# kwohlfahrt/collision

Measured on AMD Instinct MI355X. Metric: M spheres/sec end-to-end (bounds->Morton->radix sort->LBVH->refit->traversal), higher is better.
Workload: dtype f32 coords / u32 keys+ids; 1 GPU; BASELINE config 2: 1000000 uniform-random spheres, r=0.001, f32, RandomState(4), pair capacity 131072; spheres_total=1000000, group_size=256, parallelism=single

## Files before the change

### collision_amd/csrc/bvh.hip

```cpp
#include "col_common.h"
#include <math.h>

namespace {

constexpr u32 END = 0xFFFFFFFFu;

template <typename T> struct BTypes;
template <> struct BTypes<float> {
    typedef float4 V4;
    typedef uint32_t Bits;
    struct alignas(4) V3 { float x, y, z; };
};
template <> struct BTypes<double> {
    typedef double4 V4;
    typedef uint64_t Bits;
    struct alignas(8) V3 { double x, y, z; };
};

template <typename T> __device__ __forceinline__ u32 link_load(const T *bounds, uint64_t row) {
    typedef typename BTypes<T>::Bits Bits;
    return (u32) reinterpret_cast<const Bits *>(bounds)[row * 4 + 3];
}
template <typename T> __device__ __forceinline__ void link_store(T *bounds, uint64_t row, u32 v) {
    typedef typename BTypes<T>::Bits Bits;
// ... 1076 lines not shown
    if (coord_bytes != 4 && coord_bytes != 8) return COL_EINVAL;
    if (n_dev && !partials) return COL_EINVAL;
    if (partials && (parts == 0 || parts > COL_MINMAX_PARTS)) return COL_EINVAL;
    if (padded < n || (capacity > 0 && !pairs)) return COL_EINVAL;
    if (!scratch) return COL_ENOSCRATCH;
    if (col_radix_tile_override_active()) return COL_EINVAL;
    hipStream_t s = col_stream(stream);
    if (n == 0) {
        COL_HIP(hipMemsetAsync(counter, 0, sizeof(uint32_t), s));
        return COL_OK;
    }
    (void)flags;
    char *p = (char *)scratch;
    void *range = p;           p += 256;
    void *red_scratch = p;     p += col_reduce_scratch_bytes(coord_bytes == 8 ? COL_F64 : COL_F32, 4);
    p = (char *)(((uintptr_t)p + 255) & ~(uintptr_t)255);
    void *sort_scratch = p;    p += col_radix_scratch_bytes(padded, 4, 4);
    p = (char *)(((uintptr_t)p + 255) & ~(uintptr_t)255);
    void *lbvh_scratch = p;    p += col_lbvh_scratch_bytes(n, coord_bytes);
    p = (char *)(((uintptr_t)p + 255) & ~(uintptr_t)255);
    void *packed = p;          p += (size_t)n * 4 * coord_bytes;
    p = (char *)(((uintptr_t)p + 255) & ~(uintptr_t)255);
    void *chunk_hdr = p;       p += sizeof(ChunkHdr) + 256 + 8 * ((size_t)n / 64 + 1) + 256;
    p = (char *)(((uintptr_t)p + 255) & ~(uintptr_t)255);
    uint32_t *msd_fused = (uint32_t *)p;
    const bool chunked = (sort_plan & COL_TRAVERSE_CHUNKED) != 0;
    sort_plan &= 1;
    uint32_t *publish = oversize ? oversize + 2 : nullptr;
    int rc;
    uint32_t *report_word = nullptr;
    const uint32_t tile = col_radix_tile(padded, 4, 4);
    if (tile == 1024 || tile == 4096 || tile == 8192) {
        const bool msd = sort_plan == COL_SORT_MSD && padded <= COL_MSD_MAX_N;
        const uint32_t nsums = msd ? (uint32_t)(col_radix_msd_fused_bytes() / sizeof(uint32_t)) : 0u;
        if (msd && col_ceil_div(padded, tile) > (uint64_t)COL_MSD_GROUP * COL_MSD_GROUPS) return COL_EINVAL;
        if (!partials) {
            if ((rc = col_minmax4_stage1_zero(stream, coords, n, coord_bytes, red_scratch, &parts, msd_fused, nsums))) return rc;
            partials = red_scratch;
        } else if (msd)
            COL_HIP(hipMemsetAsync(msd_fused, 0, nsums * sizeof(uint32_t), s));
        if ((rc = col_morton_tile(stream, coords, radii, partials, parts, n, padded, coord_bytes, codes0, ids0, packed,
                                  counter, (uint32_t *)sort_scratch, tile, (uint32_t)col_ceil_div(padded, tile), msd ? 22 : 0,
                                  publish, n_dev, msd ? msd_fused : nullptr))) return rc;
        if (msd) rc = col_radix_sort_msd_fused(stream, codes0, codes1, ids0, ids1, padded, sort_scratch, oversize, n_dev, msd_fused);
        else rc = col_radix_sort_ex(stream, codes0, codes1, ids0, ids1, padded, 4, 4, sort_scratch, 0, 1);
        if (rc) return rc;
        if (!msd && oversize && padded <= COL_MSD_MAX_N) report_word = oversize + 1;
    } else {
        if (n_dev) return COL_EINVAL;
        if ((rc = col_reduce(stream, coords, n, coord_bytes == 8 ? COL_F64 : COL_F32, 4, COL_OP_MINMAX, red_scratch, range))) return rc;
        if ((rc = col_morton_ex(stream, coords, radii, range, n, padded, coord_bytes, codes0, ids0, packed, counter, publish))) return rc;
        if ((rc = col_radix_sort(stream, codes0, codes1, ids0, ids1, padded, 4, 4, sort_scratch, 0))) return rc;
    }
    uint32_t *sched = (!chunked && (n >= COL_DYNAMIC_PACKETS_FROM || (g_traverse_variant & 32768))) ? (uint32_t *)((char *)chunk_hdr + sizeof(ChunkHdr)) : nullptr;
    const int order_mode = chunked || col_lbvh_order_forced() ? 1 : 0;
    uint32_t *walk_order = n > 256 && (chunked || (sched && (n <= COL_DEAL_MAX_N || order_mode))) ? (uint32_t *)((char *)chunk_hdr + sizeof(ChunkHdr) + 256) : nullptr;
    if ((rc = col_lbvh_ex(stream, codes1, ids1, coords, radii, packed, nodes, bounds, lbvh_scratch, n, coord_bytes,
                          chunked ? (uint32_t *)chunk_hdr : sched, n_dev, walk_order, order_mode, chunked ? 16u : 8u, report_word, padded))) return rc;
    if (chunked) return traverse_chunked_dev(stream, pairs, counter, capacity, nodes, bounds, n, coord_bytes, chunk_hdr, n_dev, walk_order, true);
    if (n < 2) return COL_OK;
    if (coord_bytes == 4) return launch_traverse<float>(stream, pairs, counter, capacity, bounds, n, nullptr, 0, sched, n_dev, walk_order);
    return launch_traverse<double>(stream, pairs, counter, capacity, bounds, n, nullptr, 0, sched, n_dev, walk_order);
}

}
```

### collision_amd/csrc/col_common.h

```cpp
#pragma once
#include <hip/hip_runtime.h>
#include <stdint.h>
#include "../../include/collision_hip.h"
#include "../../include/collision_hip_debug.h"

#define COL_WAVE 64

#define COL_HIP(expr)                                  \
    do {                                               \
        hipError_t e_ = (expr);                        \
        if (e_ != hipSuccess) return (int)e_;          \
    } while (0)

#define COL_LAUNCH_OK()                                \
    do {                                               \
        hipError_t e_ = hipGetLastError();             \
        if (e_ != hipSuccess) return (int)e_;          \
    } while (0)

extern "C" int col_morton_ex(void *stream, const void *coords, const void *radii, const void *range, uint32_t n,
                             uint32_t padded, int coord_bytes, uint32_t *codes, uint32_t *ids, void *packed,
                             uint32_t *zero_word, uint32_t *publish);
extern "C" int col_lbvh_ex(void *stream, const uint32_t *codes, const uint32_t *ids, const void *coords, const void *radii,
                           const void *packed, col_node *nodes, void *bounds, void *scratch, uint32_t n, int coord_bytes,
                           uint32_t *zero8,
                           const uint32_t *n_dev,
                           uint32_t *walk_order,
                           int order_mode,
                           uint32_t nzero = 8,
                           uint32_t *report_word = nullptr,
                           uint32_t report_n = 0);
extern "C" int col_radix_sort_msd_dev(void *stream, const uint32_t *keys, uint32_t *keys_out, const uint32_t *vals, uint32_t *vals_out,
                                      uint64_t n, void *scratch, uint32_t *oversize, const uint32_t *n_real_dev);

#define COL_MINMAX_PARTS 256
#define COL_REGION_BOXES 8
#define COL_MSD_SMALL_N 1900000u
#define COL_MSD_MAX_N 4050000u
extern "C" int col_minmax4_stage1(void *stream, const void *rows, uint64_t n, int coord_bytes, void *partials, uint32_t *parts);
extern "C" int col_minmax4_stage1_dev(void *stream, const void *rows, const uint32_t *n_dev, uint32_t n_max, int coord_bytes,
                                      void *partials, uint32_t *parts);
extern "C" int col_morton_tile(void *stream, const void *coords, const void *radii, const void *partials, uint32_t parts,
                               uint32_t n, uint32_t padded, int coord_bytes, uint32_t *codes, uint32_t *ids, void *packed,
                               uint32_t *zero_word, uint32_t *hist0, uint32_t tile, uint32_t nblocks, int hist_shift,
                               uint32_t *publish, const uint32_t *n_dev, uint32_t *gsum);
#define COL_MSD_GROUP 32u
#define COL_MSD_GROUPS 32u
extern "C" int col_minmax4_stage1_zero(void *stream, const void *rows, uint64_t n, int coord_bytes, void *partials, uint32_t *parts,
                                       uint32_t *zero, uint32_t nzero);
extern "C" size_t col_radix_msd_fused_bytes(void);
extern "C" int col_radix_sort_msd_fused(void *stream, const uint32_t *keys, uint32_t *keys_out, const uint32_t *vals, uint32_t *vals_out,
                                        uint64_t n, void *scratch, uint32_t *oversize, const uint32_t *n_real_dev, uint32_t *fused);
extern "C" int col_radix_sort_ex(void *stream, const void *keys, void *keys_out, const void *vals, void *vals_out,
                                 uint64_t n, int key_bytes, int val_bytes, void *scratch, int copy_back, int have_hist0);

extern "C" int col_traverse_ghost_packets(void *stream, uint32_t *pairs, uint32_t *counter, uint32_t capacity, const void *bounds,
                                          uint32_t n, int coord_bytes, const uint32_t *rec, const uint32_t *order,
                                          const uint32_t *count, uint32_t max_ghosts, const uint32_t *local_gids,
                                          const uint32_t *n_dev);
extern "C" int col_radix_sort_low_passes(void *stream, const uint32_t *keys, uint32_t *keys_out, const uint32_t *vals,
                                         uint32_t *vals_out, uint64_t n, void *scratch, int passes);
extern "C" int col_radix_bucket_report(void *stream, const uint32_t *sorted_codes, uint64_t n, uint32_t *word);

static inline hipStream_t col_stream(void *s) { return (hipStream_t)s; }

static inline uint64_t col_ceil_div(uint64_t a, uint64_t b) { return (a + b - 1) / b; }

#ifdef __HIPCC__
typedef unsigned long long u64;
typedef unsigned int u32;
__device__ __forceinline__ void col_bucket_report_block(const u32 *__restrict__ sorted, u32 n, u32 *word, u32 *s_start) {
    const u32 d = threadIdx.x;
    const u32 want = d << 22;
    u32 lo = 0, hi = n;
    while (lo < hi) {
        const u32 mid = lo + ((hi - lo) >> 1);
        if (sorted[mid] < want) lo = mid + 1; else hi = mid;
    }
    s_start[d] = lo;
    if (d == 0) {
        u32 l2 = 0, h2 = n;
        while (l2 < h2) {
            const u32 mid = l2 + ((h2 - l2) >> 1);
            if (sorted[mid] < (1u << 30)) l2 = mid + 1; else h2 = mid;
        }
        s_start[256] = l2;
    }
    __syncthreads();
    u32 cnt = s_start[d + 1] - s_start[d];
#pragma unroll
    for (int o = COL_WAVE / 2; o > 0; o >>= 1) cnt = max(cnt, (u32)__shfl_xor((int)cnt, o, COL_WAVE));
    __syncthreads();
    if ((d & 63u) == 0) s_start[d >> 6] = cnt;
    __syncthreads();
    if (d == 0) {
        const u32 m = max(max(s_start[0], s_start[1]), max(s_start[2], s_start[3]));
        __hip_atomic_store(word, 0x80000000u | min(m, 0x7FFFFFFFu), __ATOMIC_RELAXED, __HIP_MEMORY_SCOPE_SYSTEM);
    }
}

__device__ __forceinline__ u32 lane_id() { return __lane_id(); }

__device__ __forceinline__ u32 count_of(u32 n, const u32 *__restrict__ n_dev) { return n_dev ? min(n, *n_dev) : n; }

__device__ __forceinline__ u32 mbcnt(u64 mask) {
    return __builtin_amdgcn_mbcnt_hi((u32)(mask >> 32), __builtin_amdgcn_mbcnt_lo((u32)mask, 0u));
}

__device__ __forceinline__ u32 wave_incl_scan(u32 v) {
    const u32 lane = lane_id();
#pragma unroll
    for (int o = 1; o < COL_WAVE; o <<= 1) {
        u32 t = __shfl_up(v, o, COL_WAVE);
        if (lane >= (u32)o) v += t;
    }
    return v;
}

__device__ __forceinline__ u32 wave_sum(u32 v) {
#pragma unroll
    for (int o = COL_WAVE / 2; o > 0; o >>= 1) v += __shfl_xor(v, o, COL_WAVE);
    return v;
}

template <int NT>
__device__ __forceinline__ u32 block_excl_scan(u32 v, u32 *warp_sums, u32 *total) {
    constexpr int NW = NT / COL_WAVE;
    const u32 lane = lane_id(), w = threadIdx.x / COL_WAVE;
    u32 incl = wave_incl_scan(v);
    if (lane == COL_WAVE - 1) warp_sums[w] = incl;
    __syncthreads();
    u32 base = 0, tot = 0;
#pragma unroll
    for (int i = 0; i < NW; i++) {
        u32 s = warp_sums[i];
        if ((u32)i < w) base += s;
        tot += s;
    }
    __syncthreads();
// ... 46 lines not shown
```

### collision_amd/csrc/morton.hip

```cpp
#include "col_common.h"

namespace {


template <typename T> struct alignas(4 * sizeof(T)) Vec4 { T x, y, z, w; };
template <> struct alignas(16) Vec4<double> { double x, y, z, w; };

__device__ __forceinline__ void publish_count(u32 *publish, u32 count) {
    if (publish) __hip_atomic_store(publish, 0x80000000u | (count < 0x7FFFFFFFu ? count : 0x7FFFFFFFu), __ATOMIC_RELAXED, __HIP_MEMORY_SCOPE_SYSTEM);
}

template <typename T>
__global__ __launch_bounds__(256) void k_morton(const Vec4<T> *__restrict__ coords,
                                                 const Vec4<T> *__restrict__ range, u32 n, u32 padded,
                                                 u32 *__restrict__ codes, u32 *__restrict__ ids,
                                                 const T *__restrict__ radii, Vec4<T> *__restrict__ packed,
                                                 u32 *__restrict__ zero_word, u32 *publish) {
    const u32 i = blockIdx.x * 256 + threadIdx.x;
    if (i == 0 && zero_word) {
        publish_count(publish, *zero_word);
        *zero_word = 0;
    }
    if (i >= padded) return;
    u32 code = 0xFFFFFFFFu;
    if (i < n) {
        const Vec4<T> mn = range[0], mx = range[1];
        const Vec4<T> c = coords[i];
        if (packed) {
            Vec4<T> pr = c;
            pr.w = radii[i];
            packed[i] = pr;
        }
        code = (expand_bits(quantize(c.x, mn.x, mx.x)) << 2) + (expand_bits(quantize(c.y, mn.y, mx.y)) << 1) +
               expand_bits(quantize(c.z, mn.z, mx.z));
    }
    codes[i] = code;
    if (ids) ids[i] = i;
}

constexpr int MT_ROWS = 4;
template <typename T, int NT, int HALVES>
__global__ __launch_bounds__(NT) void k_morton_tile(const Vec4<T> *__restrict__ coords, const T *__restrict__ partials,
                                                     u32 parts, u32 n_bound, u32 padded, u32 *__restrict__ codes,
                                                     u32 *__restrict__ ids, const T *__restrict__ radii,
                                                     Vec4<T> *__restrict__ packed, u32 *__restrict__ zero_word,
                                                     u32 *__restrict__ hist0, u32 nblocks, int hist_shift, u32 *publish,
                                                     const u32 *__restrict__ n_dev, u32 *__restrict__ gsum) {
    constexpr int TILE = NT * MT_ROWS * HALVES, NW = NT / 64;
    const u32 n = count_of(n_bound, n_dev);
    __shared__ T s_fold[NW][8];
    __shared__ u32 s_hist[256];
    const u32 tid = threadIdx.x, lane = tid & 63u, w = tid >> 6;
    if (blockIdx.x == 0 && tid == 0 && zero_word) {
        publish_count(publish, *zero_word);
        *zero_word = 0;
    }
    if (tid < 256) s_hist[tid] = 0;
    Vec4<T> c[MT_ROWS];
    T rad[MT_ROWS];
#pragma unroll
    for (int k = 0; k < MT_ROWS; k++) {
        const u32 i = blockIdx.x * TILE + k * NT + tid;
        if (i < n) {
            c[k] = coords[i];
            if (packed) rad[k] = radii[i];
        }
    }
    T acc[8];
#pragma unroll
    for (int k = 0; k < 4; k++) { acc[k] = (T)INFINITY; acc[4 + k] = -(T)INFINITY; }
    for (u32 i = tid; i < parts; i += NT) {
        const T *q = partials + (size_t)i * 8;
#pragma unroll
        for (int k = 0; k < 4; k++) {
            acc[k] = q[k] < acc[k] ? q[k] : acc[k];
            acc[4 + k] = q[4 + k] > acc[4 + k] ? q[4 + k] : acc[4 + k];
        }
    }
#pragma unroll
    for (int o = 32; o > 0; o >>= 1) {
#pragma unroll
        for (int k = 0; k < 4; k++) {
            const T lo = __shfl_xor(acc[k], o, 64), hi = __shfl_xor(acc[4 + k], o, 64);
            acc[k] = lo < acc[k] ? lo : acc[k];
            acc[4 + k] = hi > acc[4 + k] ? hi : acc[4 + k];
        }
    }
    if (lane == 0) {
#pragma unroll
        for (int k = 0; k < 8; k++) s_fold[w][k] = acc[k];
    }
    __syncthreads();
    Vec4<T> mn, mx;
    {
        T r[8];
#pragma unroll
        for (int k = 0; k < 8; k++) r[k] = s_fold[0][k];
        for (int ww = 1; ww < NW; ww++) {
#pragma unroll
            for (int k = 0; k < 4; k++) {
                r[k] = s_fold[ww][k] < r[k] ? s_fold[ww][k] : r[k];
                r[4 + k] = s_fold[ww][4 + k] > r[4 + k] ? s_fold[ww][4 + k] : r[4 + k];
            }
        }
        mn.x = r[0]; mn.y = r[1]; mn.z = r[2]; mn.w = r[3];
        mx.x = r[4]; mx.y = r[5]; mx.z = r[6]; mx.w = r[7];
    }
#pragma unroll
    for (int h = 0; h < HALVES; h++) {
        if (h > 0) {
#pragma unroll
            for (int k = 0; k < MT_ROWS; k++) {
                const u32 i = blockIdx.x * TILE + (h * MT_ROWS + k) * NT + tid;
                if (i < n) {
                    c[k] = coords[i];
                    if (packed) rad[k] = radii[i];
                }
            }
        }
#pragma unroll
        for (int k = 0; k < MT_ROWS; k++) {
            const u32 i = blockIdx.x * TILE + (h * MT_ROWS + k) * NT + tid;
            if (i >= padded) continue;
            u32 code = 0xFFFFFFFFu;
            if (i < n) {
                if (packed) {
                    Vec4<T> pr = c[k];
                    pr.w = rad[k];
                    packed[i] = pr;
                }
                code = (expand_bits(quantize(c[k].x, mn.x, mx.x)) << 2) + (expand_bits(quantize(c[k].y, mn.y, mx.y)) << 1) +
                       expand_bits(quantize(c[k].z, mn.z, mx.z));
            }
            codes[i] = code;
            if (ids) ids[i] = i;
            atomicAdd(&s_hist[(code >> hist_shift) & 255u], 1u);
        }
    }
    __syncthreads();
    if (gsum) {
        if (tid < 256) {
            const u32 c = s_hist[tid];
            hist0[(uint64_t)blockIdx.x * 256 + tid] = c;
            if (c) atomicAdd(&gsum[(blockIdx.x / COL_MSD_GROUP) * 256 + tid], c);
        }
        return;
    }
    if (tid < 256) hist0[(uint64_t)tid * nblocks + blockIdx.x] = s_hist[tid];
}

template <typename T>
int launch_morton_tile(hipStream_t s, u32 tile, const void *coords, const void *radii, const void *partials, uint32_t parts,
                       uint32_t n, uint32_t padded, uint32_t *codes, uint32_t *ids, void *packed, uint32_t *zero_word,
                       uint32_t *hist0, uint32_t nblocks, int hist_shift, uint32_t *publish, const uint32_t *n_dev, uint32_t *gsum) {
    dim3 grid(nblocks);
    if (tile == 1024)
        k_morton_tile<T, 256, 1><<<grid, dim3(256), 0, s>>>((const Vec4<T> *)coords, (const T *)partials, parts, n, padded, codes, ids,
                                                             (const T *)radii, (Vec4<T> *)packed, zero_word, hist0, nblocks, hist_shift, publish, n_dev, gsum);
    else if (tile == 4096)
        k_morton_tile<T, 1024, 1><<<grid, dim3(1024), 0, s>>>((const Vec4<T> *)coords, (const T *)partials, parts, n, padded, codes, ids,
                                                               (const T *)radii, (Vec4<T> *)packed, zero_word, hist0, nblocks, hist_shift, publish, n_dev, gsum);
    else
        k_morton_tile<T, 1024, 2><<<grid, dim3(1024), 0, s>>>((const Vec4<T> *)coords, (const T *)partials, parts, n, padded, codes, ids,
                                                               (const T *)radii, (Vec4<T> *)packed, zero_word, hist0, nblocks, hist_shift, publish, n_dev, gsum);
    COL_LAUNCH_OK();
    return COL_OK;
}

}

extern "C" {

int col_morton_tile(void *stream, const void *coords, const void *radii, const void *partials, uint32_t parts,
                    uint32_t n, uint32_t padded, int coord_bytes, uint32_t *codes, uint32_t *ids, void *packed,
                    uint32_t *zero_word, uint32_t *hist0, uint32_t tile, uint32_t nblocks, int hist_shift, uint32_t *publish,
                    const uint32_t *n_dev, uint32_t *gsum) {
    if (padded < n || parts == 0 || !hist0 || hist_shift < 0 || hist_shift > 24) return COL_EINVAL;
    if (tile != 1024 && tile != 4096 && tile != 8192) return COL_EINVAL;
    if (padded == 0) return COL_OK;
    if (packed && !radii) return COL_EINVAL;
    if (nblocks != (uint32_t)col_ceil_div(padded, tile)) return COL_EINVAL;
    if (coord_bytes == 4)
        return launch_morton_tile<float>(col_stream(stream), tile, coords, radii, partials, parts, n, padded, codes, ids, packed,
                                         zero_word, hist0, nblocks, hist_shift, publish, n_dev, gsum);
    if (coord_bytes == 8)
        return launch_morton_tile<double>(col_stream(stream), tile, coords, radii, partials, parts, n, padded, codes, ids, packed,
                                          zero_word, hist0, nblocks, hist_shift, publish, n_dev, gsum);
    return COL_EINVAL;
}

int col_morton_ex(void *stream, const void *coords, const void *radii, const void *range, uint32_t n, uint32_t padded,
                  int coord_bytes, uint32_t *codes, uint32_t *ids, void *packed, uint32_t *zero_word, uint32_t *publish) {
    if (padded < n) return COL_EINVAL;
    if (padded == 0) return COL_OK;
    if (packed && !radii) return COL_EINVAL;
    dim3 grid((unsigned)col_ceil_div(padded, 256)), block(256);
    if (coord_bytes == 4)
        k_morton<float><<<grid, block, 0, col_stream(stream)>>>((const Vec4<float> *)coords, (const Vec4<float> *)range, n, padded,
                                                                codes, ids, (const float *)radii, (Vec4<float> *)packed, zero_word, publish);
    else if (coord_bytes == 8)
        k_morton<double><<<grid, block, 0, col_stream(stream)>>>((const Vec4<double> *)coords, (const Vec4<double> *)range, n,
                                                                 padded, codes, ids, (const double *)radii, (Vec4<double> *)packed,
                                                                 zero_word, publish);
    else
        return COL_EINVAL;
    COL_LAUNCH_OK();
    return COL_OK;
}

int col_morton(void *stream, const void *coords, const void *range, uint32_t n, uint32_t padded, int coord_bytes,
               uint32_t *codes, uint32_t *ids) {
    return col_morton_ex(stream, coords, nullptr, range, n, padded, coord_bytes, codes, ids, nullptr, nullptr, nullptr);
}

}
```

### collision_amd/csrc/radix.hip

```cpp
#include "col_common.h"
#include <algorithm>

namespace {

constexpr int RT = 256;
constexpr int RDIG = 256;
constexpr int BS_SHIFT_REPORT = 22;
constexpr int IT_BIG = 16, IT_SMALL = 4, IT_HUGE = 32;
constexpr int NT_BIG = 512, NT_MID = 256, NT_SMALL = 256, NT_HUGE = 512;
constexpr uint64_t SMALL_N = 1u << 20, BIG_N = 8u << 20, HUGE_N = 32u << 20;
constexpr int HG = 16;

template <int B> struct Val;
template <> struct Val<4> { typedef uint32_t T; };
template <> struct Val<8> { typedef uint2 T; };
template <> struct Val<16> { typedef uint4 T; };
struct alignas(16) V32 { uint4 a, b; };
template <> struct Val<32> { typedef V32 T; };

template <typename K> __device__ __forceinline__ u32 digit_of(K key, int shift) { return (u32)(key >> shift) & (RDIG - 1); }

__device__ __forceinline__ u64 match8(u32 d) {
    u32 m[8];
    u64 bal[8];
#pragma unroll
    for (int b = 0; b < 8; b++) {
        m[b] = (u32)__builtin_amdgcn_sbfe(d, b, 1);
        asm("" : "+v"(m[b]));
    }
#pragma unroll
    for (int b = 0; b < 8; b++) bal[b] = __builtin_amdgcn_ballot_w64(m[b] != 0);
    u32 dlo = 0, dhi = 0;
#pragma unroll
    for (int b = 0; b < 8; b++) {
        dlo = __builtin_amdgcn_bitop3_b32(dlo, (u32)bal[b], m[b], 0xF6);
        dhi = __builtin_amdgcn_bitop3_b32(dhi, (u32)(bal[b] >> 32), m[b], 0xF6);
    }
    return ~(((u64)dhi << 32) | dlo);
}

constexpr int HC = 16;
template <typename K, int TILE>
__global__ __launch_bounds__(RT) __attribute__((amdgpu_num_sgpr(80))) void k_hist(const K *__restrict__ keys, uint64_t n, u32 nblocks, u32 g,
                                             int shift, u32 *__restrict__ hist) {
    constexpr int IT = TILE / RT;
    constexpr int VEC = 16 / sizeof(K);
    constexpr int NV = IT / VEC;
    __shared__ __attribute__((aligned(16))) u32 col[RDIG * HC];
    __shared__ u32 h[HG * RDIG];
    typedef u32 v4u __attribute__((ext_vector_type(4)));
    const u32 tid = threadIdx.x, c = tid & (HC - 1);
#pragma unroll
    for (int j = 0; j < HC / 4; j++) *reinterpret_cast<v4u *>(col + tid * HC + 4 * j) = v4u{0, 0, 0, 0};
    __syncthreads();
    const u32 b0 = blockIdx.x * g;
    const u32 cnt = min(g, nblocks - b0);
    const u32 m = cnt && (uint64_t)(b0 + cnt) * TILE > n ? cnt - 1 : cnt;
    auto issue = [&](v4u (&dst)[NV], uint64_t base) {
#pragma unroll
        for (int k = 0; k < NV; k++)
            asm volatile("global_load_dwordx4 %0, %1, off" : "=v"(dst[k]) : "v"(keys + base + ((uint64_t)k * RT + tid) * VEC) : "memory");
    };
    auto arrived = [&](v4u (&dst)[NV]) {
#pragma unroll
        for (int k = 0; k < NV; k++) asm volatile("s_waitcnt vmcnt(0)" : "+v"(dst[k])::"memory");
    };
    auto fold = [&](u32 t) {
        __syncthreads();
        u32 sum = 0;
#pragma unroll
        for (int j = 0; j < HC / 4; j++) {
            v4u *p = reinterpret_cast<v4u *>(col + tid * HC + 4 * ((j + (tid >> 2)) & (HC / 4 - 1)));
// ... 344 lines not shown
    }
}

constexpr int BS_NT = 1024, BS_NW = BS_NT / COL_WAVE;
constexpr int BS_SHIFT = 22;

template <int BS_IT> struct BucketLds {
    u32 keys[BS_NT * BS_IT];
    u32 vals[BS_NT * BS_IT];
    u32 cnt[BS_NW][RDIG];
    u32 base[RDIG];
    u32 ws[BS_NW];
};

template <int BS_IT>
__device__ __forceinline__ void bucket_rank(BucketLds<BS_IT> &lds, const u32 (&key)[BS_IT], u32 (&pos)[BS_IT], u32 m, int shift,
                                            u32 w, u32 tid, u32 row_len) {
    for (u32 i = tid; i < BS_NW * RDIG; i += BS_NT) (&lds.cnt[0][0])[i] = 0;
    __syncthreads();
#pragma unroll
    for (int k = 0; k < BS_IT; k++) {
        pos[k] = 0;
        if ((u32)k * COL_WAVE >= row_len || w * row_len + k * COL_WAVE >= m) continue;
        const u32 d = digit_of(key[k], shift);
        const u64 peers = match8(d);
        const u32 below = mbcnt(peers);
        const u32 prev = lds.cnt[w][d];
        if (below == 0) lds.cnt[w][d] = prev + (u32)__popcll(peers);
        pos[k] = prev + below;
    }
    __syncthreads();
}

template <int BS_IT>
__global__ __launch_bounds__(BS_NT) void k_bucket_sort(u32 *__restrict__ k_a, u32 *__restrict__ v_a, u32 *__restrict__ k_b,
                                                        u32 *__restrict__ v_b, u32 n, const u32 *__restrict__ offsets,
                                                        u32 nblocks, u32 *oversize, const u32 *__restrict__ n_real_dev) {
    constexpr u32 BS_CAP = BS_NT * BS_IT;
    constexpr int BS_ROW = COL_WAVE * BS_IT;
    __shared__ BucketLds<BS_IT> lds;
    const u32 tid = threadIdx.x, lane = tid & (COL_WAVE - 1);
    const u32 w = (u32)__builtin_amdgcn_readfirstlane((int)(tid / COL_WAVE));
    const u32 d = blockIdx.x;
    const u32 start = offsets[(uint64_t)d * nblocks], end = d + 1 < RDIG ? offsets[(uint64_t)(d + 1) * nblocks] : n;
    u32 pads = 0;
    if (n_real_dev) {
        const u32 n_real = min(n, *n_real_dev), all = n - n_real, per = (all + RDIG - 1) / RDIG;
        for (u32 i = threadIdx.x; i < per; i += BS_NT) {
            const u32 j = n_real + d * per + i;
            if (j < n) { k_b[j] = 0xFFFFFFFFu; v_b[j] = j; }
        }
        if (d == RDIG - 1) pads = min(end - start, all);
    }
    const u32 S = end - start - pads;
    if (S == 0) return;
    u32 key[BS_IT], val[BS_IT], pos[BS_IT];

    if (S <= BS_CAP) {
        const u32 L = ((S + BS_NW - 1) / BS_NW + COL_WAVE - 1) & ~(u32)(COL_WAVE - 1);
#pragma unroll
        for (int k = 0; k < BS_IT; k++) {
            const u32 p = w * L + k * COL_WAVE + lane;
            const bool ok = (u32)k * COL_WAVE < L && p < S;
            key[k] = ok ? k_a[start + p] : 0xFFFFFFFFu;
            val[k] = ok ? v_a[start + p] : 0u;
        }
        for (int shift = 0; shift < BS_SHIFT; shift += 8) {
            bucket_rank<BS_IT>(lds, key, pos, S, shift, w, tid, L);
            {
                u32 c[BS_NW], tot = 0;
                if (tid < RDIG) {
#pragma unroll
                    for (int i = 0; i < BS_NW; i++) { c[i] = lds.cnt[i][tid]; tot += c[i]; }
                }
                u32 total;
                const u32 dstart = block_excl_scan<BS_NT>(tot, lds.ws, &total);
                if (tid < RDIG) {
                    u32 run = dstart;
#pragma unroll
                    for (int i = 0; i < BS_NW; i++) { lds.cnt[i][tid] = run; run += c[i]; }
                }
            }
            __syncthreads();
#pragma unroll
            for (int k = 0; k < BS_IT; k++) {
                if ((u32)k * COL_WAVE >= L || w * L + k * COL_WAVE >= S) continue;
                const u32 q = pos[k] + lds.cnt[w][digit_of(key[k], shift)];
                lds.keys[q] = key[k];
                lds.vals[q] = val[k];
            }
            __syncthreads();
#pragma unroll
            for (int k = 0; k < BS_IT; k++) {
                const u32 p = w * L + k * COL_WAVE + lane;
                if ((u32)k * COL_WAVE >= L || w * L + k * COL_WAVE >= S) continue;
                key[k] = p < S ? lds.keys[p] : 0xFFFFFFFFu;
                val[k] = p < S ? lds.vals[p] : 0u;
            }
        }
#pragma unroll
        for (int k = 0; k < BS_IT; k++) {
            const u32 p = w * L + k * COL_WAVE + lane;
            if ((u32)k * COL_WAVE < L && p < S) { k_b[start + p] = key[k]; v_b[start + p] = val[k]; }
        }
        return;
    }

    if (tid == 0 && oversize) *oversize = S;
    int pass = 0;
    for (int shift = 0; shift < BS_SHIFT; shift += 8, pass++) {
        const u32 *sk = ((pass & 1) ? k_b : k_a) + start, *sv = ((pass & 1) ? v_b : v_a) + start;
        u32 *dk = ((pass & 1) ? k_a : k_b) + start, *dv = ((pass & 1) ? v_a : v_b) + start;
        if (tid < RDIG) lds.base[tid] = 0;
        __syncthreads();
        for (u32 i = tid; i < S; i += BS_NT) atomicAdd(&lds.base[digit_of(sk[i], shift)], 1u);
        __syncthreads();
        {
            u32 total;
            const u32 mine = tid < RDIG ? lds.base[tid] : 0u;
            const u32 ex = block_excl_scan<BS_NT>(mine, lds.ws, &total);
            if (tid < RDIG) lds.base[tid] = ex;
        }
        __syncthreads();
        for (u32 c0 = 0; c0 < S; c0 += BS_CAP) {
            const u32 m = min(BS_CAP, S - c0);
#pragma unroll
            for (int k = 0; k < BS_IT; k++) {
                const u32 p = w * BS_ROW + k * COL_WAVE + lane;
                key[k] = p < m ? sk[c0 + p] : 0xFFFFFFFFu;
                val[k] = p < m ? sv[c0 + p] : 0u;
            }
            bucket_rank<BS_IT>(lds, key, pos, m, shift, w, tid, (u32)BS_ROW);
            if (tid < RDIG) {
                u32 run = lds.base[tid];
#pragma unroll
                for (int i = 0; i < BS_NW; i++) { const u32 c = lds.cnt[i][tid]; lds.cnt[i][tid] = run; run += c; }
                if (tid == RDIG - 1) {
                    const u32 ranked = ((m + COL_WAVE - 1) / COL_WAVE) * COL_WAVE;
                    run -= ranked - m;
                }
                lds.base[tid] = run;
            }
            __syncthreads();
#pragma unroll
            for (int k = 0; k < BS_IT; k++) {
// ... 360 lines not shown
        k_bucket_sort<8><<<dim3(RDIG), dim3(BS_NT), 0, s>>>(tmp_keys, tmp_vals, keys_out, vals_out, (u32)n, hist, (u32)nb, oversize, n_real_dev);
    else
        k_bucket_sort<16><<<dim3(RDIG), dim3(BS_NT), 0, s>>>(tmp_keys, tmp_vals, keys_out, vals_out, (u32)n, hist, (u32)nb, oversize, n_real_dev);
    COL_LAUNCH_OK();
    return COL_OK;
}

size_t col_radix_msd_fused_bytes(void) { return (size_t)(MSD_GROUPS + 1) * RDIG * sizeof(u32); }
int col_radix_sort_msd_fused(void *stream, const uint32_t *keys, uint32_t *keys_out, const uint32_t *vals, uint32_t *vals_out,
                             uint64_t n, void *scratch, uint32_t *oversize, const uint32_t *n_real_dev, uint32_t *fused) {
    if (n == 0) return COL_OK;
    if (!scratch || !vals || !vals_out || !fused) return COL_EINVAL;
    if (n > COL_MSD_MAX_N) return COL_EINVAL;
    const u32 tile = tile_auto(n, 4, 4);
    hipStream_t s = col_stream(stream);
    const size_t nb = col_ceil_div(n, tile);
    if (nb > (size_t)MSD_GROUP * MSD_GROUPS) return COL_EINVAL;
    char *p = (char *)scratch;
    const u32 *counts = (const u32 *)p; p += align256((size_t)RDIG * nb * sizeof(u32));
    p += align256(col_scan_scratch_bytes((uint64_t)RDIG * nb));
    u32 *tmp_keys = (u32 *)p;          p += align256((size_t)n * 4);
    u32 *tmp_vals = (u32 *)p;
    u32 *starts = fused + MSD_GROUPS * RDIG;
    const FusedOn f{fused, starts};
    if (tile == (u32)(NT_SMALL * IT_SMALL))
        k_scatter<u32, 4, IT_SMALL, NT_SMALL, true><<<dim3((unsigned)nb), dim3(NT_SMALL), 0, s>>>(keys, tmp_keys, vals, tmp_vals, n, (u32)nb, BS_SHIFT, counts, f);
    else
        k_scatter<u32, 4, IT_BIG, NT_MID, true><<<dim3((unsigned)nb), dim3(NT_MID), 0, s>>>(keys, tmp_keys, vals, tmp_vals, n, (u32)nb, BS_SHIFT, counts, f);
    COL_LAUNCH_OK();
    if (n <= COL_MSD_SMALL_N)
        k_bucket_sort<8><<<dim3(RDIG), dim3(BS_NT), 0, s>>>(tmp_keys, tmp_vals, keys_out, vals_out, (u32)n, starts, 1u, oversize, n_real_dev);
    else
        k_bucket_sort<16><<<dim3(RDIG), dim3(BS_NT), 0, s>>>(tmp_keys, tmp_vals, keys_out, vals_out, (u32)n, starts, 1u, oversize, n_real_dev);
    COL_LAUNCH_OK();
    return COL_OK;
}

static int sort_passes(void *stream, const void *keys, void *keys_out, const void *vals, void *vals_out,
                       uint64_t n, int key_bytes, int val_bytes, void *scratch, int copy_back, int have_hist0, int passes);
int col_radix_sort_low_passes(void *stream, const uint32_t *keys, uint32_t *keys_out, const uint32_t *vals,
                              uint32_t *vals_out, uint64_t n, void *scratch, int passes) {
    if (passes < 1 || passes > 4) return COL_EINVAL;
    return sort_passes(stream, keys, keys_out, vals, vals_out, n, 4, 4, scratch, 0, 0, passes);
}

int col_radix_bucket_report(void *stream, const uint32_t *sorted_codes, uint64_t n, uint32_t *word) {
    if (!sorted_codes || !word || n == 0 || n >= 0xFFFFFFFFull) return COL_EINVAL;
    k_bucket_report<<<dim3(1), dim3(RDIG), 0, col_stream(stream)>>>(sorted_codes, (u32)n, word);
    COL_LAUNCH_OK();
    return COL_OK;
}

int col_radix_sort(void *stream, const void *keys, void *keys_out, const void *vals, void *vals_out,
                   uint64_t n, int key_bytes, int val_bytes, void *scratch, int copy_back) {
    return col_radix_sort_ex(stream, keys, keys_out, vals, vals_out, n, key_bytes, val_bytes, scratch, copy_back, 0);
}

static int sort_passes(void *stream, const void *keys, void *keys_out, const void *vals, void *vals_out,
                       uint64_t n, int key_bytes, int val_bytes, void *scratch, int copy_back, int have_hist0, int passes);

int col_radix_sort_ex(void *stream, const void *keys, void *keys_out, const void *vals, void *vals_out,
                      uint64_t n, int key_bytes, int val_bytes, void *scratch, int copy_back, int have_hist0) {
    if (!vals || !vals_out) val_bytes = 0;
    if (narrow_key(key_bytes)) {
        if (n >= 0xFFFFFFFFull || have_hist0 || !(native_value(val_bytes) || wide_value(val_bytes))) return COL_EINVAL;
        if (n == 0) return COL_OK;
// ... 118 lines not shown
```

### collision_amd/csrc/runtime.hip

```cpp
#include "col_common.h"
#include <string.h>

namespace {

template <typename T>
__global__ void k_fill(T *dst, T v, size_t count) {
    size_t i = (size_t)blockIdx.x * blockDim.x + threadIdx.x;
    const size_t stride = (size_t)gridDim.x * blockDim.x;
    for (; i < count; i += stride) dst[i] = v;
}

template <typename T>
static int fill_launch(void *stream, void *dst, const void *pattern, size_t count) {
    T v;
    memcpy(&v, pattern, sizeof(T));
    size_t blocks = col_ceil_div(count, 256);
    if (blocks > 4096) blocks = 4096;
    k_fill<T><<<dim3((unsigned)blocks), dim3(256), 0, col_stream(stream)>>>((T *)dst, v, count);
    COL_LAUNCH_OK();
    return COL_OK;
}

__global__ void k_xcc_census(unsigned *out) {
    if (threadIdx.x == 0) out[blockIdx.x] = __builtin_amdgcn_s_getreg((3 << 11) | 20) & 0xF;
}

}

extern "C" {

int col_debug_xcc_census(void *stream, uint32_t *out, uint32_t nblocks) {
    k_xcc_census<<<dim3(nblocks), dim3(256), 0, col_stream(stream)>>>(out);
    COL_LAUNCH_OK();
    return COL_OK;
}

const char *col_error_string(int code) {
    if (code == COL_OK) return "ok";
    if (code == COL_EINVAL) return "collision_hip: invalid argument";
    if (code == COL_ENOSCRATCH) return "collision_hip: missing scratch buffer";
    if (code > 0) return hipGetErrorString((hipError_t)code);
    return "collision_hip: unknown error";
}

int col_version(void) { return 101; }

int col_device_count(int *count) { COL_HIP(hipGetDeviceCount(count)); return COL_OK; }
int col_set_device(int device) { COL_HIP(hipSetDevice(device)); return COL_OK; }
int col_get_device(int *device) { COL_HIP(hipGetDevice(device)); return COL_OK; }
int col_device_sync(void) { COL_HIP(hipDeviceSynchronize()); return COL_OK; }

int col_device_name(char *buf, int len) {
    int dev = 0;
    hipDeviceProp_t prop;
    COL_HIP(hipGetDevice(&dev));
    COL_HIP(hipGetDeviceProperties(&prop, dev));
    if (len <= 0) return COL_EINVAL;
    snprintf(buf, (size_t)len, "%s %s (%d CUs)", prop.name, prop.gcnArchName, prop.multiProcessorCount);
    return COL_OK;
}

int col_malloc(void **ptr, size_t bytes) { COL_HIP(hipMalloc(ptr, bytes ? bytes : 4)); return COL_OK; }
int col_free(void *ptr) { COL_HIP(hipFree(ptr)); return COL_OK; }
int col_host_alloc(void **ptr, size_t bytes) { COL_HIP(hipHostMalloc(ptr, bytes ? bytes : 4, hipHostMallocCoherent)); return COL_OK; }
int col_host_free(void *ptr) { COL_HIP(hipHostFree(ptr)); return COL_OK; }

int col_memcpy_h2d(void *stream, void *dst, const void *src, size_t bytes) {
    if (bytes) COL_HIP(hipMemcpyAsync(dst, src, bytes, hipMemcpyHostToDevice, col_stream(stream)));
    return COL_OK;
}
int col_memcpy_d2h(void *stream, void *dst, const void *src, size_t bytes) {
    if (bytes) COL_HIP(hipMemcpyAsync(dst, src, bytes, hipMemcpyDeviceToHost, col_stream(stream)));
    return COL_OK;
}
int col_memcpy_d2d(void *stream, void *dst, const void *src, size_t bytes) {
    if (bytes) COL_HIP(hipMemcpyAsync(dst, src, bytes, hipMemcpyDeviceToDevice, col_stream(stream)));
    return COL_OK;
}
// ... 46 lines not shown
```

Measured before the change: 7091 M spheres/s.

## Locally sort Morton tiles by top digit and gather buckets in MSD sort

The Morton kernel gets a sorted mode that ranks each tile's keys by the top 8-bit digit in LDS and writes them back grouped by digit, together with a per-tile (offset,count) table and group sums. A new MSD bucket-sort variant then has each digit block gather its contiguous runs from every tile with vectorized loads, instead of needing a separate scatter pass into digit buckets. For large inputs the Morton tile grows to 4096. This removes a global scatter and the separate offset scan, at the cost of extra LDS work in the Morton kernel, more complex gather logic, and an extra overflow buffer path.

```diff
diff --git a/collision_amd/csrc/bvh.hip b/collision_amd/csrc/bvh.hip
--- a/collision_amd/csrc/bvh.hip
+++ b/collision_amd/csrc/bvh.hip
@@ -1132,6 +1132,8 @@
     const uint32_t tile = col_radix_tile(padded, 4, 4);
     if (tile == 1024 || tile == 4096 || tile == 8192) {
         const bool msd = sort_plan == COL_SORT_MSD && padded <= COL_MSD_MAX_N;
+        const bool gather = msd && tile == 1024;
+        const uint32_t mtile = gather && padded >= COL_GATHER_BIG_FROM ? 4096u : tile;
         const uint32_t nsums = msd ? (uint32_t)(col_radix_msd_fused_bytes() / sizeof(uint32_t)) : 0u;
         if (msd && col_ceil_div(padded, tile) > (uint64_t)COL_MSD_GROUP * COL_MSD_GROUPS) return COL_EINVAL;
         if (!partials) {
@@ -1140,9 +1142,10 @@
         } else if (msd)
             COL_HIP(hipMemsetAsync(msd_fused, 0, nsums * sizeof(uint32_t), s));
         if ((rc = col_morton_tile(stream, coords, radii, partials, parts, n, padded, coord_bytes, codes0, ids0, packed,
-                                  counter, (uint32_t *)sort_scratch, tile, (uint32_t)col_ceil_div(padded, tile), msd ? 22 : 0,
-                                  publish, n_dev, msd ? msd_fused : nullptr))) return rc;
-        if (msd) rc = col_radix_sort_msd_fused(stream, codes0, codes1, ids0, ids1, padded, sort_scratch, oversize, n_dev, msd_fused);
+                                  counter, (uint32_t *)sort_scratch, mtile, (uint32_t)col_ceil_div(padded, mtile), msd ? 22 : 0,
+                                  publish, n_dev, msd ? msd_fused : nullptr, gather ? 1 : 0))) return rc;
+        if (gather) rc = col_radix_sort_msd_gather(stream, codes0, codes1, ids0, ids1, n, padded, sort_scratch, oversize, n_dev, msd_fused, mtile);
+        else if (msd) rc = col_radix_sort_msd_fused(stream, codes0, codes1, ids0, ids1, padded, sort_scratch, oversize, n_dev, msd_fused);
         else rc = col_radix_sort_ex(stream, codes0, codes1, ids0, ids1, padded, 4, 4, sort_scratch, 0, 1);
         if (rc) return rc;
         if (!msd && oversize && padded <= COL_MSD_MAX_N) report_word = oversize + 1;
diff --git a/collision_amd/csrc/col_common.h b/collision_amd/csrc/col_common.h
--- a/collision_amd/csrc/col_common.h
+++ b/collision_amd/csrc/col_common.h
@@ -43,7 +43,12 @@
 extern "C" int col_morton_tile(void *stream, const void *coords, const void *radii, const void *partials, uint32_t parts,
                                uint32_t n, uint32_t padded, int coord_bytes, uint32_t *codes, uint32_t *ids, void *packed,
                                uint32_t *zero_word, uint32_t *hist0, uint32_t tile, uint32_t nblocks, int hist_shift,
-                               uint32_t *publish, const uint32_t *n_dev, uint32_t *gsum);
+                               uint32_t *publish, const uint32_t *n_dev, uint32_t *gsum,
+                               int sorted);
+extern "C" int col_radix_sort_msd_gather(void *stream, const uint32_t *tile_keys, uint32_t *keys_out, const uint32_t *tile_vals,
+                                         uint32_t *vals_out, uint32_t n_bound, uint64_t padded, void *scratch, uint32_t *oversize,
+                                         const uint32_t *n_dev, const uint32_t *gsum, uint32_t tile);
+#define COL_GATHER_BIG_FROM (768u << 10)
 #define COL_MSD_GROUP 32u
 #define COL_MSD_GROUPS 32u
 extern "C" int col_minmax4_stage1_zero(void *stream, const void *rows, uint64_t n, int coord_bytes, void *partials, uint32_t *parts,
@@ -105,6 +110,25 @@
 
 __device__ __forceinline__ u32 mbcnt(u64 mask) {
     return __builtin_amdgcn_mbcnt_hi((u32)(mask >> 32), __builtin_amdgcn_mbcnt_lo((u32)mask, 0u));
+}
+
+__device__ __forceinline__ u64 match8(u32 d) {
+    u32 m[8];
+    u64 bal[8];
+#pragma unroll
+    for (int b = 0; b < 8; b++) {
+        m[b] = (u32)__builtin_amdgcn_sbfe(d, b, 1);
+        asm("" : "+v"(m[b]));
+    }
+#pragma unroll
+    for (int b = 0; b < 8; b++) bal[b] = __builtin_amdgcn_ballot_w64(m[b] != 0);
+    u32 dlo = 0, dhi = 0;
+#pragma unroll
+    for (int b = 0; b < 8; b++) {
+        dlo = __builtin_amdgcn_bitop3_b32(dlo, (u32)bal[b], m[b], 0xF6);
+        dhi = __builtin_amdgcn_bitop3_b32(dhi, (u32)(bal[b] >> 32), m[b], 0xF6);
+    }
+    return ~(((u64)dhi << 32) | dlo);
 }
 
 __device__ __forceinline__ u32 wave_incl_scan(u32 v) {
diff --git a/collision_amd/csrc/morton.hip b/collision_amd/csrc/morton.hip
--- a/collision_amd/csrc/morton.hip
+++ b/collision_amd/csrc/morton.hip
@@ -39,7 +39,7 @@
 }
 
 constexpr int MT_ROWS = 4;
-template <typename T, int NT, int HALVES>
+template <typename T, int NT, int HALVES, bool SORTED = false>
 __global__ __launch_bounds__(NT) void k_morton_tile(const Vec4<T> *__restrict__ coords, const T *__restrict__ partials,
                                                      u32 parts, u32 n_bound, u32 padded, u32 *__restrict__ codes,
                                                      u32 *__restrict__ ids, const T *__restrict__ radii,
@@ -51,16 +51,18 @@
     __shared__ T s_fold[NW][8];
     __shared__ u32 s_hist[256];
     const u32 tid = threadIdx.x, lane = tid & 63u, w = tid >> 6;
+    static_assert(!SORTED || (HALVES == 1 && NT >= 256), "the sorted tile: a thread per digit, one pass");
+    auto row_of = [&](int k) -> u32 { return SORTED ? w * (64u * MT_ROWS) + (u32)k * 64u + lane : (u32)k * NT + tid; };
     if (blockIdx.x == 0 && tid == 0 && zero_word) {
         publish_count(publish, *zero_word);
         *zero_word = 0;
     }
-    if (tid < 256) s_hist[tid] = 0;
+    if constexpr (!SORTED) { if (tid < 256) s_hist[tid] = 0; }
     Vec4<T> c[MT_ROWS];
     T rad[MT_ROWS];
 #pragma unroll
     for (int k = 0; k < MT_ROWS; k++) {
-        const u32 i = blockIdx.x * TILE + k * NT + tid;
+        const u32 i = blockIdx.x * TILE + row_of(k);
         if (i < n) {
             c[k] = coords[i];
             if (packed) rad[k] = radii[i];
@@ -105,6 +107,77 @@
         }
         mn.x = r[0]; mn.y = r[1]; mn.z = r[2]; mn.w = r[3];
         mx.x = r[4]; mx.y = r[5]; mx.z = r[6]; mx.w = r[7];
+    }
+    if constexpr (SORTED) {
+        __shared__ __attribute__((aligned(16))) u32 s_k[TILE], s_i[TILE];
+        __shared__ u32 s_cnt[NW][256];
+        __shared__ u32 s_ws[NW];
+        typedef u32 v4u __attribute__((ext_vector_type(4)));
+        const u32 base = blockIdx.x * TILE;
+        for (u32 i = lane; i < 256; i += 64) s_cnt[w][i] = 0;
+        __builtin_amdgcn_wave_barrier();
+        u32 code[MT_ROWS], pos[MT_ROWS];
+#pragma unroll
+        for (int k = 0; k < MT_ROWS; k++) {
+            const u32 i = base + row_of(k);
+            code[k] = 0xFFFFFFFFu;
+            if (i < n) {
+                if (packed) {
+                    Vec4<T> pr = c[k];
+                    pr.w = rad[k];
+                    packed[i] = pr;
+                }
+                code[k] = (expand_bits(quantize(c[k].x, mn.x, mx.x)) << 2) + (expand_bits(quantize(c[k].y, mn.y, mx.y)) << 1) +
+                          expand_bits(quantize(c[k].z, mn.z, mx.z));
+            }
+        }
+#pragma unroll
+        for (int k = 0; k < MT_ROWS; k++) {
+            const u32 d = (code[k] >> hist_shift) & 255u;
+            const u64 peers = match8(d);
+            const u32 below = mbcnt(peers);
+            const u32 prev = s_cnt[w][d];
+            if (below == 0) s_cnt[w][d] = prev + (u32)__popcll(peers);
+            pos[k] = prev + below;
+        }
+        __syncthreads();
+        {
+            u32 cw[NW], tot = 0;
+            if (tid < 256) {
+#pragma unroll
+                for (int i = 0; i < NW; i++) { cw[i] = s_cnt[i][tid]; tot += cw[i]; }
+            }
+            u32 total;
+            const u32 dstart = block_excl_scan<NT>(tot, s_ws, &total);
+            if (tid < 256) {
+                u32 run = dstart;
+#pragma unroll
+                for (int i = 0; i < NW; i++) { s_cnt[i][tid] = run; run += cw[i]; }
+                const u32 real = n > base ? min(n - base, (u32)TILE) : 0u;
+                const u32 cnt = tid == 255u ? tot - ((u32)TILE - real) : tot;
+                hist0[(uint64_t)blockIdx.x * 256 + tid] = dstart << 16 | cnt;
+                if (cnt) atomicAdd(&gsum[(blockIdx.x / COL_MSD_GROUP) * 256 + tid], cnt);
+            }
+        }
+        __syncthreads();
+#pragma unroll
+        for (int k = 0; k < MT_ROWS; k++) {
+            const u32 q = pos[k] + s_cnt[w][(code[k] >> hist_shift) & 255u];
+            s_k[q] = code[k];
+            s_i[q] = base + row_of(k);
+        }
+        __syncthreads();
+        if (base + TILE <= padded && (((uintptr_t)codes | (uintptr_t)ids) & 15u) == 0) {
+            reinterpret_cast<v4u *>(codes + base)[tid] = reinterpret_cast<const v4u *>(s_k)[tid];
+            reinterpret_cast<v4u *>(ids + base)[tid] = reinterpret_cast<const v4u *>(s_i)[tid];
+        } else {
+#pragma unroll
+            for (int k = 0; k < MT_ROWS; k++) {
+                const u32 q = (u32)k * NT + tid;
+                if (base + q < padded) { codes[base + q] = s_k[q]; ids[base + q] = s_i[q]; }
+            }
+        }
+        return;
     }
 #pragma unroll
     for (int h = 0; h < HALVES; h++) {
@@ -152,9 +225,15 @@
 template <typename T>
 int launch_morton_tile(hipStream_t s, u32 tile, const void *coords, const void *radii, const void *partials, uint32_t parts,
                        uint32_t n, uint32_t padded, uint32_t *codes, uint32_t *ids, void *packed, uint32_t *zero_word,
-                       uint32_t *hist0, uint32_t nblocks, int hist_shift, uint32_t *publish, const uint32_t *n_dev, uint32_t *gsum) {
+                       uint32_t *hist0, uint32_t nblocks, int hist_shift, uint32_t *publish, const uint32_t *n_dev, uint32_t *gsum, int sorted) {
     dim3 grid(nblocks);
-    if (tile == 1024)
+    if (sorted && tile == 4096)
+        k_morton_tile<T, 1024, 1, true><<<grid, dim3(1024), 0, s>>>((const Vec4<T> *)coords, (const T *)partials, parts, n, padded, codes, ids,
+                                                                     (const T *)radii, (Vec4<T> *)packed, zero_word, hist0, nblocks, hist_shift, publish, n_dev, gsum);
+    else if (sorted)
+        k_morton_tile<T, 256, 1, true><<<grid, dim3(256), 0, s>>>((const Vec4<T> *)coords, (const T *)partials, parts, n, padded, codes, ids,
+                                                                   (const T *)radii, (Vec4<T> *)packed, zero_word, hist0, nblocks, hist_shift, publish, n_dev, gsum);
+    else if (tile == 1024)
         k_morton_tile<T, 256, 1><<<grid, dim3(256), 0, s>>>((const Vec4<T> *)coords, (const T *)partials, parts, n, padded, codes, ids,
                                                              (const T *)radii, (Vec4<T> *)packed, zero_word, hist0, nblocks, hist_shift, publish, n_dev, gsum);
     else if (tile == 4096)
@@ -174,7 +253,8 @@
 int col_morton_tile(void *stream, const void *coords, const void *radii, const void *partials, uint32_t parts,
                     uint32_t n, uint32_t padded, int coord_bytes, uint32_t *codes, uint32_t *ids, void *packed,
                     uint32_t *zero_word, uint32_t *hist0, uint32_t tile, uint32_t nblocks, int hist_shift, uint32_t *publish,
-                    const uint32_t *n_dev, uint32_t *gsum) {
+                    const uint32_t *n_dev, uint32_t *gsum, int sorted) {
+    if (sorted && ((tile != 1024 && tile != 4096) || !gsum || !ids || !codes)) return COL_EINVAL;
     if (padded < n || parts == 0 || !hist0 || hist_shift < 0 || hist_shift > 24) return COL_EINVAL;
     if (tile != 1024 && tile != 4096 && tile != 8192) return COL_EINVAL;
     if (padded == 0) return COL_OK;
@@ -182,10 +262,10 @@
     if (nblocks != (uint32_t)col_ceil_div(padded, tile)) return COL_EINVAL;
     if (coord_bytes == 4)
         return launch_morton_tile<float>(col_stream(stream), tile, coords, radii, partials, parts, n, padded, codes, ids, packed,
-                                         zero_word, hist0, nblocks, hist_shift, publish, n_dev, gsum);
+                                         zero_word, hist0, nblocks, hist_shift, publish, n_dev, gsum, sorted);
     if (coord_bytes == 8)
         return launch_morton_tile<double>(col_stream(stream), tile, coords, radii, partials, parts, n, padded, codes, ids, packed,
-                                          zero_word, hist0, nblocks, hist_shift, publish, n_dev, gsum);
+                                          zero_word, hist0, nblocks, hist_shift, publish, n_dev, gsum, sorted);
     return COL_EINVAL;
 }
 
diff --git a/collision_amd/csrc/radix.hip b/collision_amd/csrc/radix.hip
--- a/collision_amd/csrc/radix.hip
+++ b/collision_amd/csrc/radix.hip
@@ -20,24 +20,6 @@
 
 template <typename K> __device__ __forceinline__ u32 digit_of(K key, int shift) { return (u32)(key >> shift) & (RDIG - 1); }
 
-__device__ __forceinline__ u64 match8(u32 d) {
-    u32 m[8];
-    u64 bal[8];
-#pragma unroll
-    for (int b = 0; b < 8; b++) {
-        m[b] = (u32)__builtin_amdgcn_sbfe(d, b, 1);
-        asm("" : "+v"(m[b]));
-    }
-#pragma unroll
-    for (int b = 0; b < 8; b++) bal[b] = __builtin_amdgcn_ballot_w64(m[b] != 0);
-    u32 dlo = 0, dhi = 0;
-#pragma unroll
-    for (int b = 0; b < 8; b++) {
-        dlo = __builtin_amdgcn_bitop3_b32(dlo, (u32)bal[b], m[b], 0xF6);
-        dhi = __builtin_amdgcn_bitop3_b32(dhi, (u32)(bal[b] >> 32), m[b], 0xF6);
-    }
-    return ~(((u64)dhi << 32) | dlo);
-}
 
 constexpr int HC = 16;
 template <typename K, int TILE>
@@ -448,28 +430,131 @@
     __syncthreads();
 }
 
-template <int BS_IT>
+constexpr u32 GATHER_CHUNKS = 4, GATHER_GLOG_MAX = 4;
+__host__ __device__ constexpr u32 gather_piece(u32 glog) { return ((4u * GATHER_CHUNKS) << glog) - 3u; }
+struct GatherOff {};
+struct GatherOn { const u32 *gsum; u32 n_bound; u32 tile; u32 glog; u32 *x_keys, *x_vals; };
+template <bool GATHER> struct GatherArg { typedef GatherOff T; };
+template <> struct GatherArg<true> { typedef GatherOn T; };
+template <bool GATHER> __device__ __forceinline__ u32 *oversize_area(u32 *a, const typename GatherArg<GATHER>::T &ga, bool keys) {
+    if constexpr (GATHER) return keys ? ga.x_keys : ga.x_vals; else return a;
+}
+
+template <int BS_IT, bool GATHER = false>
 __global__ __launch_bounds__(BS_NT) void k_bucket_sort(u32 *__restrict__ k_a, u32 *__restrict__ v_a, u32 *__restrict__ k_b,
                                                         u32 *__restrict__ v_b, u32 n, const u32 *__restrict__ offsets,
-                                                        u32 nblocks, u32 *oversize, const u32 *__restrict__ n_real_dev) {
+                                                        u32 nblocks, u32 *oversize, const u32 *__restrict__ n_real_dev,
+                                                        typename GatherArg<GATHER>::T ga = {}) {
     constexpr u32 BS_CAP = BS_NT * BS_IT;
     constexpr int BS_ROW = COL_WAVE * BS_IT;
     __shared__ BucketLds<BS_IT> lds;
     const u32 tid = threadIdx.x, lane = tid & (COL_WAVE - 1);
     const u32 w = (u32)__builtin_amdgcn_readfirstlane((int)(tid / COL_WAVE));
-    const u32 d = blockIdx.x;
-    const u32 start = offsets[(uint64_t)d * nblocks], end = d + 1 < RDIG ? offsets[(uint64_t)(d + 1) * nblocks] : n;
-    u32 pads = 0;
-    if (n_real_dev) {
-        const u32 n_real = min(n, *n_real_dev), all = n - n_real, per = (all + RDIG - 1) / RDIG;
-        for (u32 i = threadIdx.x; i < per; i += BS_NT) {
-            const u32 j = n_real + d * per + i;
-            if (j < n) { k_b[j] = 0xFFFFFFFFu; v_b[j] = j; }
-        }
-        if (d == RDIG - 1) pads = min(end - start, all);
-    }
-    const u32 S = end - start - pads;
-    if (S == 0) return;
+    const u32 d = GATHER ? (blockIdx.x & 7u) * (RDIG / 8) + (blockIdx.x >> 3) : blockIdx.x;
+    u32 start, S;
+    if constexpr (GATHER) {
+        static_assert(BS_NT >= MSD_GROUP * MSD_GROUPS && BS_NT == 4 * RDIG, "one thread per tile; four threads per digit column of the group sums");
+        u32 *const l_src = &lds.cnt[0][0], *const l_pos = l_src + BS_NT, *const l_cnt = l_src + 2 * BS_NT;
+        u32 *const l_n = &lds.base[BS_NW];
+        const u32 glog = ga.glog, sub = tid & ((1u << glog) - 1u), my_tile = tid >> glog;
+        const u32 word = my_tile < nblocks ? offsets[(uint64_t)my_tile * RDIG + d] : 0u;
+        const u32 ngroups = (nblocks + MSD_GROUP - 1) / MSD_GROUP;
+        u32 below = 0;
+        {
+            const u32 j = tid & (RDIG - 1), g0 = tid / RDIG;
+#pragma unroll
+            for (int m = 0; m < MSD_GROUPS / 4; m++) {
+                const u32 g = g0 + 4u * m;
+                if (j < d && g < ngroups) below += ga.gsum[g * RDIG + j];
+            }
+        }
+        const u32 n_real = count_of(min(ga.n_bound, n), n_real_dev);
+        if (tid == 0) *l_n = 0;
+        {
+            const u32 all = n - n_real, per = (all + RDIG - 1) / RDIG;
+            for (u32 i = tid; i < per; i += BS_NT) {
+                const u32 j = n_real + d * per + i;
+                if (j < n) { k_b[j] = 0xFFFFFFFFu; v_b[j] = j; }
+            }
+        }
+        const u32 g_cnt = word & 0xFFFFu, g_src = my_tile * ga.tile + (word >> 16);
+        u32 g_pos;
+        {
+            const u32 one = sub == 0 ? g_cnt : 0u;
+            const u32 incl = wave_incl_scan(one), bs = wave_sum(below);
+            if (lane == COL_WAVE - 1) lds.ws[w] = incl;
+            if (lane == 0) lds.base[w] = bs;
+            __syncthreads();
+            u32 pre = 0, tot = 0, st = 0;
+#pragma unroll
+            for (int i = 0; i < BS_NW; i++) {
+                const u32 s = lds.ws[i];
+                if ((u32)i < w) pre += s;
+                tot += s;
+                st += lds.base[i];
+            }
+            g_pos = (u32)__shfl((int)(pre + incl - one), (int)(lane & ~((1u << glog) - 1u)), COL_WAVE);
+            S = tot;
+            start = st;
+        }
+        if (S == 0) return;
+        if (start + S > n_real) return;
+        const bool fits = S <= BS_CAP;
+        u32 *const xk = ga.x_keys + start, *const xv = ga.x_vals + start;
+        typedef u32 v4u __attribute__((ext_vector_type(4)));
+        const u32 a0 = g_src & ~3u, sh = g_src & 3u;
+        const bool mine = g_cnt <= gather_piece(glog) && a0 + ((sh + g_cnt + 3u) & ~3u) <= n && (((uintptr_t)k_a | (uintptr_t)v_a) & 15u) == 0;
+        if (!mine && sub == 0 && g_cnt) {
+            const u32 e = atomicAdd(l_n, 1u);
+            l_src[e] = g_src; l_pos[e] = g_pos; l_cnt[e] = g_cnt;
+        }
+        v4u pk[GATHER_CHUNKS], pv[GATHER_CHUNKS];
+#pragma unroll
+        for (u32 c = 0; c < GATHER_CHUNKS; c++) {
+            const u32 ci = (c << glog) + sub;
+            const u32 a = mine && 4u * ci < sh + g_cnt ? a0 + 4u * ci : 0u;
+            pk[c] = *reinterpret_cast<const v4u *>(k_a + a);
+            pv[c] = *reinterpret_cast<const v4u *>(v_a + a);
+        }
+#pragma unroll
+        for (u32 c = 0; c < GATHER_CHUNKS; c++) {
+#pragma unroll
+            for (u32 i = 0; i < 4; i++) {
+                const u32 j = 4u * ((c << glog) + sub) + i - sh;
+                if (mine && j < g_cnt) {
+                    if (fits) { lds.keys[g_pos + j] = pk[c][i]; lds.vals[g_pos + j] = pv[c][i]; }
+                    else { xk[g_pos + j] = pk[c][i]; xv[g_pos + j] = pv[c][i]; }
+                }
+            }
+        }
+        __syncthreads();
+        const u32 nl = *l_n;
+        for (u32 e = w; e < nl; e += BS_NW) {
+            const u32 src = l_src[e], q = l_pos[e], c = l_cnt[e];
+            for (u32 j = lane; j < c; j += COL_WAVE) {
+                const u32 kk = k_a[src + j], vv = v_a[src + j];
+                if (fits) { lds.keys[q + j] = kk; lds.vals[q + j] = vv; }
+                else { xk[q + j] = kk; xv[q + j] = vv; }
+            }
+        }
+        if (!fits) __builtin_amdgcn_fence(__ATOMIC_RELEASE, "agent");
+        __syncthreads();
+        if (!fits) __builtin_amdgcn_fence(__ATOMIC_ACQUIRE, "agent");
+    } else {
+        start = offsets[(uint64_t)d * nblocks];
+        const u32 end = d + 1 < RDIG ? offsets[(uint64_t)(d + 1) * nblocks] : n;
+        u32 pads = 0;
+        if (n_real_dev) {
+            const u32 n_real = min(n, *n_real_dev), all = n - n_real, per = (all + RDIG - 1) / RDIG;
+            for (u32 i = threadIdx.x; i < per; i += BS_NT) {
+                const u32 j = n_real + d * per + i;
+                if (j < n) { k_b[j] = 0xFFFFFFFFu; v_b[j] = j; }
+            }
+            if (d == RDIG - 1) pads = min(end - start, all);
+        }
+        S = end - start - pads;
+        if (S == 0) return;
+    }
     u32 key[BS_IT], val[BS_IT], pos[BS_IT];
 
     if (S <= BS_CAP) {
@@ -478,8 +563,13 @@
         for (int k = 0; k < BS_IT; k++) {
             const u32 p = w * L + k * COL_WAVE + lane;
             const bool ok = (u32)k * COL_WAVE < L && p < S;
-            key[k] = ok ? k_a[start + p] : 0xFFFFFFFFu;
-            val[k] = ok ? v_a[start + p] : 0u;
+            if constexpr (GATHER) {
+                key[k] = ok ? lds.keys[p] : 0xFFFFFFFFu;
+                val[k] = ok ? lds.vals[p] : 0u;
+            } else {
+                key[k] = ok ? k_a[start + p] : 0xFFFFFFFFu;
+                val[k] = ok ? v_a[start + p] : 0u;
+            }
         }
         for (int shift = 0; shift < BS_SHIFT; shift += 8) {
             bucket_rank<BS_IT>(lds, key, pos, S, shift, w, tid, L);
@@ -523,10 +613,11 @@
     }
 
     if (tid == 0 && oversize) *oversize = S;
+    u32 *const o_k = oversize_area<GATHER>(k_a, ga, true), *const o_v = oversize_area<GATHER>(v_a, ga, false);
     int pass = 0;
     for (int shift = 0; shift < BS_SHIFT; shift += 8, pass++) {
-        const u32 *sk = ((pass & 1) ? k_b : k_a) + start, *sv = ((pass & 1) ? v_b : v_a) + start;
-        u32 *dk = ((pass & 1) ? k_a : k_b) + start, *dv = ((pass & 1) ? v_a : v_b) + start;
+        const u32 *sk = ((pass & 1) ? k_b : o_k) + start, *sv = ((pass & 1) ? v_b : o_v) + start;
+        u32 *dk = ((pass & 1) ? o_k : k_b) + start, *dv = ((pass & 1) ? o_v : v_b) + start;
         if (tid < RDIG) lds.base[tid] = 0;
         __syncthreads();
         for (u32 i = tid; i < S; i += BS_NT) atomicAdd(&lds.base[digit_of(sk[i], shift)], 1u);
@@ -953,6 +1044,28 @@
         k_bucket_sort<8><<<dim3(RDIG), dim3(BS_NT), 0, s>>>(tmp_keys, tmp_vals, keys_out, vals_out, (u32)n, starts, 1u, oversize, n_real_dev);
     else
         k_bucket_sort<16><<<dim3(RDIG), dim3(BS_NT), 0, s>>>(tmp_keys, tmp_vals, keys_out, vals_out, (u32)n, starts, 1u, oversize, n_real_dev);
+    COL_LAUNCH_OK();
+    return COL_OK;
+}
+
+int col_radix_sort_msd_gather(void *stream, const uint32_t *tile_keys, uint32_t *keys_out, const uint32_t *tile_vals, uint32_t *vals_out,
+                              uint32_t n_bound, uint64_t padded, void *scratch, uint32_t *oversize, const uint32_t *n_dev,
+                              const uint32_t *gsum, uint32_t tile) {
+    if (padded == 0) return COL_OK;
+    if (!scratch || !tile_keys || !tile_vals || !keys_out || !vals_out || !gsum || n_bound > padded) return COL_EINVAL;
+    if ((tile != 1024 && tile != 4096) || tile < tile_auto(padded, 4, 4) || padded > COL_MSD_SMALL_N) return COL_EINVAL;
+    const size_t nb = col_ceil_div(padded, tile);
+    if (nb > (size_t)MSD_GROUP * MSD_GROUPS || nb > (size_t)BS_NT) return COL_EINVAL;
+    u32 glog = 0;
+    while (glog < GATHER_GLOG_MAX && (nb << (glog + 1)) <= (size_t)BS_NT) glog++;
+    char *p = (char *)scratch;
+    const u32 *table = (const u32 *)p; p += align256((size_t)RDIG * nb * sizeof(u32));
+    p += align256(col_scan_scratch_bytes((uint64_t)RDIG * nb));
+    u32 *x_keys = (u32 *)p;            p += align256((size_t)padded * 4);
+    u32 *x_vals = (u32 *)p;
+    const GatherOn ga{gsum, n_bound, tile, glog, x_keys, x_vals};
+    k_bucket_sort<8, true><<<dim3(RDIG), dim3(BS_NT), 0, col_stream(stream)>>>((u32 *)tile_keys, (u32 *)tile_vals, keys_out, vals_out, (u32)padded,
+                                                                                table, (u32)nb, oversize, n_dev, ga);
     COL_LAUNCH_OK();
     return COL_OK;
 }
diff --git a/collision_amd/csrc/runtime.hip b/collision_amd/csrc/runtime.hip
--- a/collision_amd/csrc/runtime.hip
+++ b/collision_amd/csrc/runtime.hip
@@ -43,7 +43,7 @@
     return "collision_hip: unknown error";
 }
 
-int col_version(void) { return 101; }
+int col_version(void) { return 102; }
 
 int col_device_count(int *count) { COL_HIP(hipGetDeviceCount(count)); return COL_OK; }
 int col_set_device(int device) { COL_HIP(hipSetDevice(device)); return COL_OK; }
```

New measurement: 7321 M spheres/s (median of 6 runs). 3.2% higher.
